# arnauqb/GradABM-JUNE

Hardware: AMD Instinct MI355X
Metric: simulation steps/sec (higher is better)
Workload: dtype f32

## Files before the change

### gradabm-june_amd/csrc/gj_tiled.h

```cpp
#pragma once
#include <hip/hip_runtime.h>
#include <stdint.h>

#include <type_traits>

#include "../../include/gradjune_hip.h"
#include "gj_device.h"

namespace gj {

constexpr int kTileThreads = 1024;
constexpr int kTileWaves = kTileThreads / kWave;
constexpr int kMaxSliceAgents = 19840;
constexpr int kUnroll = 8;
#ifndef GJ_UNROLL_NARROW
#define GJ_UNROLL_NARROW 16
#endif
constexpr int kUnrollNarrow = GJ_UNROLL_NARROW;
#ifndef GJ_VENUE_UNROLL
#define GJ_VENUE_UNROLL 2
#endif
constexpr int kVenueUnroll = GJ_VENUE_UNROLL;
#ifndef GJ_VENUE_UNROLL_C
#define GJ_VENUE_UNROLL_C GJ_VENUE_UNROLL
#endif
constexpr int kVenueUnrollC = GJ_VENUE_UNROLL_C;
#ifndef GJ_CUM_BATCH
#define GJ_CUM_BATCH 8
#endif
constexpr int kCumBatch = GJ_CUM_BATCH;

typedef unsigned long long fx_t;
template <int BITS>
__device__ __forceinline__ constexpr float fx_max() { return (float)(1ull << (50 - BITS)); }
template <int BITS>
__device__ __forceinline__ fx_t to_fx(float x) {
  constexpr double scale = (double)(1ull << BITS);
  constexpr double magic = 6755399441055744.0;
  const double d = __builtin_fma((double)x, scale, magic);
  return (fx_t)(__double_as_longlong(d) - 0x4338000000000000LL);
}
template <int BITS>
__device__ __forceinline__ float from_fx(fx_t v) {
  return (float)((double)(long long)v * (1.0 / (double)(1ull << BITS)));
}
constexpr float kSaturated = 1.0e30f;
__device__ __forceinline__ void fx_flag(uint32_t* flags, int words, int i, float x) {
  const uint32_t bit = 1u << (i & 31);
  if (!(x < 0.0f)) atomicOr(&flags[i >> 5], bit);
  if (!(x > 0.0f)) atomicOr(&flags[words + (i >> 5)], bit);
}
__device__ __forceinline__ float fx_special(uint32_t pos, uint32_t neg, float v) {
  return (pos & neg) ? __builtin_nanf("") : (pos ? kSaturated : (neg ? -kSaturated : v));
}
template <int BITS>
__device__ __forceinline__ float fx_read(const fx_t* sums, const uint32_t* flags, int words, int i) {
  const uint32_t pos = (flags[i >> 5] >> (i & 31)) & 1u, neg = (flags[words + (i >> 5)] >> (i & 31)) & 1u;
  return fx_special(pos, neg, from_fx<BITS>(sums[i]));
}
constexpr int kFxVenue = 36, kFxAgent = 32;
__device__ __forceinline__ uint32_t abs_bits(float x) { return __float_as_uint(x) & 0x7FFFFFFFu; }
template <int N>
__device__ __forceinline__ uint32_t max_abs_bits(const float (&x)[N]) {
  uint32_t m = 0u;
#pragma unroll
  for (int q = 0; q < N; ++q) m = max(m, abs_bits(x[q]));
  return m;
}
template <int BITS>
constexpr uint32_t fx_limit_bits() { return (uint32_t)(127 + 50 - BITS) << 23; }
constexpr uint32_t kAgentLimitBits = fx_limit_bits<kFxAgent>();
static_assert(kAgentLimitBits == 0x48800000u, "the pattern of fx_max<kFxAgent>() = 262144.0f");

template <typename T>
__device__ __forceinline__ T* elem32(T* base, int idx) {
  using Byte = typename std::conditional<std::is_const<T>::value, const char, char>::type;
  return reinterpret_cast<T*>(reinterpret_cast<Byte*>(base) + (uint64_t)((uint32_t)idx * (uint32_t)sizeof(T)));
}
template <typename T>
__device__ __forceinline__ T at32(const T* base, int idx) { return *elem32(base, idx); }
template <typename T>
__device__ __forceinline__ void put32(T* base, int idx, T v) { *elem32(base, idx) = v; }

typedef float gj_v4f __attribute__((ext_vector_type(4)));
typedef unsigned int gj_v4u __attribute__((ext_vector_type(4)));
typedef unsigned int gj_v2u __attribute__((ext_vector_type(2)));
template <typename T>
__device__ __forceinline__ T at32nt(const T* base, int idx) { return __builtin_nontemporal_load(elem32(base, idx)); }
template <typename T>
__device__ __forceinline__ void put32nt(T* base, int idx, T v) { __builtin_nontemporal_store(v, elem32(base, idx)); }
__device__ __forceinline__ uint4 load_nt(const uint4* p) {
  const gj_v4u v = __builtin_nontemporal_load(reinterpret_cast<const gj_v4u*>(p));
  return make_uint4(v.x, v.y, v.z, v.w);
}
__device__ __forceinline__ float4 load_nt(const float4* p) {
  const gj_v4f v = __builtin_nontemporal_load(reinterpret_cast<const gj_v4f*>(p));
  return make_float4(v.x, v.y, v.z, v.w);
}
__device__ __forceinline__ void store_nt(float4* p, float4 x) {
  gj_v4f v = {x.x, x.y, x.z, x.w};
  __builtin_nontemporal_store(v, reinterpret_cast<gj_v4f*>(p));
}
struct TSetA {
  const uint16_t* a_la;
  const int32_t* tile_sptr;
  const int32_t* tile_jpos;
  const int32_t* chunk_ptr;
  const int4* chunk_desc;
  float* val;
  int32_t J;
  int32_t active;
  int32_t raw;
  int32_t wide;
  int32_t direct;
  int32_t presum;
  const int32_t* multi_slots;
};

struct TileAArgs {
  TSetA sets[GJ_MAX_SETS];
  int32_t n_sets;
  int32_t slice_agents;
  int64_t n_agents;
  const float* trans;
// ... 245 lines not shown
    const int i = G.edge_clamped(c0, u, lane);
    la[u] = at32(T.a_la, i);
    sl[u] = at32(slots, i);
  }
}
template <int kU>
__device__ __forceinline__ void scatter_explicit(const TSetA& T, const float* lds_x, int s, int wave, int lane) {
  const Segment G(T, s);
  for (int c0 = wave * kU; c0 < G.n_chunks; c0 += kTileWaves * kU) {
    int la[kU], sl[kU];
    explicit_stage1<kU>(T, G, c0, lane, la, sl);
#pragma unroll
    for (int u = 0; u < kU; ++u)
      if (G.has(c0, u, lane)) put32(T.val, sl[u], lds_x[la[u]]);
  }
}

template <int kU>
__device__ __forceinline__ void gather_explicit(const TSetA& T, fx_t* lds_acc, uint32_t* lds_flags, int flag_words, int s,
                                                int wave, int lane) {
  const Segment G(T, s);
  for (int c0 = wave * kU; c0 < G.n_chunks; c0 += kTileWaves * kU) {
    int la[kU], sl[kU];
    explicit_stage1<kU>(T, G, c0, lane, la, sl);
    float x[kU];
#pragma unroll
    for (int u = 0; u < kU; ++u) x[u] = at32(T.val, sl[u]);
#pragma unroll
    for (int u = 0; u < kU; ++u) x[u] = G.has(c0, u, lane) ? x[u] : 0.0f;
    agent_add_batch<kU>(lds_acc, lds_flags, flag_words, la, x);
  }
}

#ifndef GJ_SCATTER_WAVES_PER_SIMD
#define GJ_SCATTER_WAVES_PER_SIMD 4
#endif
__global__ __launch_bounds__(kTileThreads, GJ_SCATTER_WAVES_PER_SIMD) void k_tile_scatter(const TileAArgs A) {
  extern __shared__ __align__(16) float lds_x[];
  const int tid = threadIdx.x;
  const int wave = __builtin_amdgcn_readfirstlane(tid / kWave), lane = tid % kWave;
  const int s = blockIdx.x;
  const int64_t base = (int64_t)s * A.slice_agents;
  const int n_local = (int)min((int64_t)A.slice_agents, A.n_agents - base);
  const bool two_sources = A.qtrans != A.trans;
  for (int pass = 0; pass < 2; ++pass) {
    if (pass == 1 && !two_sources) break;
    bool any = false;
    for (int t = 0; t < A.n_sets; ++t)
      if (A.sets[t].active && !A.sets[t].presum && (!two_sources || A.sets[t].raw == pass)) any = true;
    if (!any) continue;
    if (pass == 1) __syncthreads();
    load_slice(lds_x, pass == 0 ? A.qtrans : A.trans, base, n_local, tid);
    __syncthreads();
    for (int t = 0; t < A.n_sets; ++t) {
      const TSetA& T = A.sets[t];
      if (!T.active || T.presum || (two_sources && T.raw != pass)) continue;
      if (T.wide == 2) {
        scatter_explicit<kUnroll>(T, lds_x, s, wave, lane);
      } else if (T.wide) {
        scatter_set<true>(T, lds_x, s, wave, lane);
      } else {
        scatter_set<false>(T, lds_x, s, wave, lane);
      }
    }
  }
}

struct TSetB {
  const int32_t* blk_v0;
  const int32_t* blk_e0;
  const uint16_t* e_lv;
  const uint8_t* e_cls;
  float* val;
  const float* v_pc;
  float* cum;
  int32_t stride;
  int32_t nk;
  float beta[GJ_MAX_NETS_PER_SET];
  int32_t table[GJ_MAX_NETS_PER_SET];
  int32_t age75[GJ_MAX_NETS_PER_SET];
  int32_t leisure;
  int32_t direct;
  uint32_t term_limit;
  int32_t _pad_b;
  const uint16_t* pv_blk;
  const int32_t* blk_r0;
  const float* x;
  int64_t n_x;
};

struct TileBArgs {
  TSetB sets[GJ_MAX_SETS];
  const int32_t* work;
  const float* tables;
  int32_t day_type;
  int32_t mode;
  int32_t transpose;
  int32_t _pad;
};

struct ClassWeights {
  float l, lw;
};
__device__ __forceinline__ ClassWeights class_weights(const float* tables, int table, int age75, int day_type, int c) {
  const float l = tables[(int64_t)table * GJ_TABLE_SIZE + day_type * 200 + c];
  return {l, age75 ? l * (((c % 100) > 75) ? 1.0f : 0.0f) : l};
}
template <bool TRANSMITTING, bool RECEIVING, typename TSet>
__device__ __forceinline__ void fill_class_weights(float* transmitting, float* receiving, const TSet& T, const float* tables,
                                                   int day_type, int transpose, int tid) {
  for (int i = tid; i < T.nk * 200; i += kTileThreads) {
    const int k = i / 200, c = i % 200;
    const ClassWeights w = class_weights(tables, T.table[k], T.age75[k], day_type, c);
    if (TRANSMITTING) transmitting[i] = transpose ? w.lw : w.l;
    if (RECEIVING) receiving[i] = transpose ? w.l : w.lw;
  }
}

__device__ __noinline__ void venue_group_slow(fx_t* sums, uint32_t* vflags, int words, uint32_t limit, int base_k, int l0,
                                              int l1, int l2, int l3, int l4, int l5, int l6, int l7, float x0, float x1,
                                              float x2, float x3, float x4, float x5, float x6, float x7) {
  const int lv[8] = {l0, l1, l2, l3, l4, l5, l6, l7};
  const float x[8] = {x0, x1, x2, x3, x4, x5, x6, x7};
#pragma unroll
  for (int q = 0; q < 8; ++q) {
    if (lv[q] == 0xFFFF) continue;
    if (abs_bits(x[q]) <= limit) {
      atomicAdd(&sums[base_k + lv[q]], to_fx<kFxVenue>(x[q]));
    } else {
      fx_flag(vflags, words, base_k + lv[q], x[q]);
    }
  }
}

__device__ __forceinline__ int class_byte(uint32_t four, int j) { return (four >> (8 * j)) & 0xFF; }

struct Group8 {
  uint32_t w[4], c[2];
  float v[8];
  __device__ __forceinline__ Group8(uint4 raw, uint2 craw, float4 xa = make_float4(0.0f, 0.0f, 0.0f, 0.0f),
                                    float4 xb = make_float4(0.0f, 0.0f, 0.0f, 0.0f))
      : w{raw.x, raw.y, raw.z, raw.w}, c{craw.x, craw.y}, v{xa.x, xa.y, xa.z, xa.w, xb.x, xb.y, xb.z, xb.w} {}
  __device__ __forceinline__ int lv(int q) const { return (w[q >> 1] >> ((q & 1) * 16)) & 0xFFFF; }
  __device__ __forceinline__ float x(int q) const { return v[q]; }
  __device__ __forceinline__ int cls(int q) const { return class_byte(c[q >> 2], q & 3); }
  __device__ __forceinline__ void drop(int q) { w[q >> 1] |= 0xFFFFu << ((q & 1) * 16); }
  __device__ __forceinline__ bool one_venue() const {
    return (w[0] == w[1]) && (w[1] == w[2]) && (w[2] == w[3]) && ((w[0] >> 16) == (w[0] & 0xFFFFu)) && (lv(0) != 0xFFFF);
  }
  __device__ __forceinline__ Group8 weighted(const float* tk) const {
    Group8 g = *this;
#pragma unroll
    for (int q = 0; q < 8; ++q) g.v[q] = tk[cls(q)] * v[q];
    return g;
  }
};

#ifdef GJ_DIAG_STAMPS
constexpr int kDiagVenueSlots = 8192;
__device__ unsigned long long gj_diag_venue[3 * kDiagVenueSlots];
struct VenueStamp {
  unsigned long long t0;
  __device__ VenueStamp() : t0(__builtin_amdgcn_s_memrealtime()) {}
  __device__ ~VenueStamp() {
    if (threadIdx.x == 0 && blockIdx.x < kDiagVenueSlots) {
      gj_diag_venue[3 * blockIdx.x] = t0;
      gj_diag_venue[3 * blockIdx.x + 1] = __builtin_amdgcn_s_memrealtime();
      gj_diag_venue[3 * blockIdx.x + 2] = __builtin_amdgcn_s_getreg((31 << 11) | 20) & 0xF;
    }
  }
};
#else
struct VenueStamp {};
#endif

struct VenueItem {
  const TSetB& T;
  int tid, nk;
  int v0, nv;
  int g0, g1;
  fx_t* sums;
  float* cumf;
  float* tabs;
  uint32_t* vflags;
  int vwords;
  int dummy;
  __device__ __forceinline__ VenueItem(const TSetB& T_, int j, float* lds, int tid_)
      : T(T_), tid(tid_), nk(T_.nk), v0(T_.blk_v0[j]), nv(T_.blk_v0[j + 1] - v0), g0(T_.blk_e0[j] >> 3),
        g1(T_.blk_e0[j + 1] >> 3), sums(reinterpret_cast<fx_t*>(lds)), cumf(lds), tabs(lds + 2 * ((size_t)nk * nv + 64)),
        vflags(reinterpret_cast<uint32_t*>(tabs + (T_.leisure ? 2 * nk * 200 : 0))), vwords((nk * nv + 64 + 31) / 32),
        dummy(nk * nv + (tid_ & 63)) {}
  __device__ __forceinline__ const uint4* lv8() const { return reinterpret_cast<const uint4*>(T.e_lv); }
  __device__ __forceinline__ const uint2* cls8() const { return reinterpret_cast<const uint2*>(T.e_cls); }
  __device__ __forceinline__ float4* val4() const { return reinterpret_cast<float4*>(T.val); }
};

__device__ __forceinline__ void run_sums(const VenueItem& W, const Group8& G, int base_k, fx_t* sums, uint32_t* vflags) {
  const uint32_t kLimit = W.T.term_limit;
  static_assert(kFxVenue == 36, "term_limit is derived from 2^(50 - kFxVenue) (fill_set_b)");
  if (__builtin_expect(max_abs_bits(G.v) > kLimit, 0)) {
    venue_group_slow(sums, vflags, W.vwords, kLimit, base_k, G.lv(0), G.lv(1), G.lv(2), G.lv(3), G.lv(4), G.lv(5),
                     G.lv(6), G.lv(7), G.x(0), G.x(1), G.x(2), G.x(3), G.x(4), G.x(5), G.x(6), G.x(7));
    return;
  }
  fx_t s8 = 0;
#pragma unroll
  for (int q = 0; q < 8; ++q) {
    const fx_t f = to_fx<kFxVenue>(G.x(q));
    const bool first = (q == 0) || (G.lv(q) != G.lv(q - (q > 0)));
    s8 = first ? f : s8 + f;
    const bool last = (q == 7) || (G.lv(q + (q < 7)) != G.lv(q));
    const bool take = last && G.lv(q) != 0xFFFF;
    atomicAdd(&sums[take ? base_k + G.lv(q) : W.dummy], s8);
  }
}
__device__ __forceinline__ bool one_venue_sum(const VenueItem& W, const Group8& G, int target, fx_t* sums) {
  if (__builtin_amdgcn_ballot_w64(max_abs_bits(G.v) > W.T.term_limit) != 0ull) return false;
  fx_t s = 0;
#pragma unroll
  for (int q = 0; q < 8; ++q) s += to_fx<kFxVenue>(G.x(q));
  s = wave_sum<fx_t>(s);
  if ((W.tid & (kWave - 1)) == 0) atomicAdd(&sums[target], s);
  return true;
}

__device__ __forceinline__ void venue_zero(const VenueItem& W, fx_t* sums, uint32_t* vflags) {
  for (int i = W.tid; i < W.nk * W.nv + 64; i += kTileThreads) sums[i] = 0;
  for (int i = W.tid; i < 2 * W.vwords; i += kTileThreads) vflags[i] = 0u;
}

__device__ __forceinline__ void venue_sums_tiled(const VenueItem& W, const float* weights, fx_t* sums, uint32_t* vflags) {
  const TSetB& T = W.T;
  auto add_group = [&](const Group8& G) {
    const bool mine = G.one_venue() && (G.lv(0) == __builtin_amdgcn_readfirstlane(G.lv(0)));
    const bool one_venue = __builtin_amdgcn_ballot_w64(mine) == ~0ull;
    if (!T.leisure) {
      if (!(one_venue && one_venue_sum(W, G, G.lv(0), sums))) run_sums(W, G, 0, sums, vflags);
    } else {
      for (int k = 0; k < W.nk; ++k) {
        const Group8 Gk = G.weighted(weights + k * 200);
        if (!(one_venue && one_venue_sum(W, Gk, k * W.nv + G.lv(0), sums))) run_sums(W, Gk, k * W.nv, sums, vflags);
      }
    }
  };
  for (int g = W.g0 + W.tid; g < W.g1; g += kVenueUnroll * kTileThreads) {
    uint4 raw[kVenueUnroll];
    float4 xa[kVenueUnroll], xb[kVenueUnroll];
    uint2 craw[kVenueUnroll];
#pragma unroll
    for (int u = 0; u < kVenueUnroll; ++u) {
      const int gu = min(g + u * kTileThreads, W.g1 - 1);
      raw[u] = W.lv8()[gu];
      xa[u] = load_nt(W.val4() + 2 * gu);
      xb[u] = load_nt(W.val4() + 2 * gu + 1);
      craw[u] = T.leisure ? W.cls8()[gu] : make_uint2(0u, 0u);
    }
#pragma unroll
    for (int u = 0; u < kVenueUnroll; ++u)
      if (g + u * kTileThreads < W.g1) add_group(Group8(raw[u], craw[u], xa[u], xb[u]));
  }
}

__device__ __forceinline__ void venue_sums_runs(const VenueItem& W, int j, fx_t* sums, uint32_t* vflags) {
  const TSetB& T = W.T;
  const int r0 = T.blk_r0[j], r1 = T.blk_r0[j + 1];
  const uint4* pv8 = reinterpret_cast<const uint4*>(T.pv_blk);
  const float4* x4 = reinterpret_cast<const float4*>(T.x);
  const int ga = r0 >> 3, gb = (r1 + 7) >> 3;
  const int g_in = (int)(T.n_x >> 3);
  for (int g = ga + W.tid; g < gb; g += kVenueUnroll * kTileThreads) {
    uint4 raw[kVenueUnroll];
    float4 xa[kVenueUnroll], xb[kVenueUnroll];
#pragma unroll
    for (int u = 0; u < kVenueUnroll; ++u) {
      const int gu = min(g + u * kTileThreads, gb - 1);
      raw[u] = pv8[gu];
      if (gu < g_in) {
        xa[u] = x4[2 * gu];
        xb[u] = x4[2 * gu + 1];
      } else {
        float t[8];
#pragma unroll
        for (int q = 0; q < 8; ++q) t[q] = ((int64_t)gu * 8 + q < T.n_x) ? T.x[(int64_t)gu * 8 + q] : 0.0f;
        xa[u] = make_float4(t[0], t[1], t[2], t[3]);
        xb[u] = make_float4(t[4], t[5], t[6], t[7]);
      }
    }
#pragma unroll
    for (int u = 0; u < kVenueUnroll; ++u) {
      const int gu = g + u * kTileThreads;
      if (gu >= gb) continue;
      Group8 G(raw[u], make_uint2(0u, 0u), xa[u], xb[u]);
#pragma unroll
      for (int q = 0; q < 8; ++q) {
        const int a = gu * 8 + q;
        if (!(a >= r0 && a < r1)) G.drop(q);
      }
      run_sums(W, G, 0, sums, vflags);
    }
  }
}

__device__ __forceinline__ void venue_cum_write(const VenueItem& W, const fx_t* sums, const uint32_t* vflags, float* cumf) {
  const TSetB& T = W.T;
  for (int l0 = W.tid; l0 < W.nv; l0 += kCumBatch * kTileThreads) {
    float pc[kCumBatch];
#pragma unroll
    for (int u = 0; u < kCumBatch; ++u) pc[u] = T.v_pc[W.v0 + min(l0 + u * kTileThreads, W.nv - 1)];
    for (int k = 0; k < W.nk; ++k) {
      const float beta = T.beta[k];
#pragma unroll
      for (int u = 0; u < kCumBatch; ++u) {
        const int lv = l0 + u * kTileThreads;
        if (lv < W.nv) {
          const float c = (beta * pc[u]) * fx_read<kFxVenue>(sums, vflags, W.vwords, k * W.nv + lv);
          T.cum[(int64_t)(W.v0 + lv) * T.stride + k] = c;
          cumf[2 * (k * W.nv + lv)] = c;
        }
      }
    }
  }
}
__device__ __forceinline__ void venue_cum_read(const VenueItem& W, float* cumf) {
  const TSetB& T = W.T;
  for (int k = 0; k < W.nk; ++k) {
    for (int l0 = W.tid; l0 < W.nv; l0 += kCumBatch * kTileThreads) {
      float c[kCumBatch];
#pragma unroll
      for (int u = 0; u < kCumBatch; ++u)
        c[u] = T.cum[(int64_t)(W.v0 + min(l0 + u * kTileThreads, W.nv - 1)) * T.stride + k];
#pragma unroll
      for (int u = 0; u < kCumBatch; ++u) {
        const int lv = l0 + u * kTileThreads;
        if (lv < W.nv) cumf[2 * (k * W.nv + lv)] = c[u];
      }
    }
  }
}

__device__ __forceinline__ void venue_gather(const VenueItem& W, const float* weights, const float* cumf) {
  const TSetB& T = W.T;
  const int nk = W.nk, nv = W.nv;
  for (int g = W.g0 + W.tid; g < W.g1; g += kVenueUnrollC * kTileThreads) {
    uint4 raw[kVenueUnrollC];
    uint2 craw[kVenueUnrollC];
#pragma unroll
    for (int u = 0; u < kVenueUnrollC; ++u) {
      const int gu = min(g + u * kTileThreads, W.g1 - 1);
      raw[u] = W.lv8()[gu];
      craw[u] = T.leisure ? W.cls8()[gu] : make_uint2(0u, 0u);
    }
#pragma unroll
    for (int u = 0; u < kVenueUnrollC; ++u) {
      const int gu = g + u * kTileThreads;
      if (gu >= W.g1) continue;
      const Group8 G(raw[u], craw[u]);
      float r[8];
      if (!T.leisure) {
#pragma unroll
        for (int q = 0; q < 8; ++q) {
          const int lv = G.lv(q);
          const float c = cumf[2 * (lv != 0xFFFF ? lv : 0)];
          r[q] = (lv != 0xFFFF) ? c : 0.0f;
        }
      } else {
#pragma unroll
        for (int q = 0; q < 8; ++q) {
          const int lv = G.lv(q);
          const int c = G.cls(q);
          const int li = lv != 0xFFFF ? lv : 0;
          float a = 0.0f;
          for (int k = 0; k < nk; ++k) a += weights[k * 200 + c] * cumf[2 * (k * nv + li)];
          r[q] = (lv != 0xFFFF) ? a : 0.0f;
        }
      }
      store_nt(W.val4() + 2 * gu, make_float4(r[0], r[1], r[2], r[3]));
      store_nt(W.val4() + 2 * gu + 1, make_float4(r[4], r[5], r[6], r[7]));
    }
  }
}

#ifndef GJ_VENUE_WAVES_PER_SIMD
#define GJ_VENUE_WAVES_PER_SIMD 4
#endif
__global__ __launch_bounds__(kTileThreads, GJ_VENUE_WAVES_PER_SIMD) void k_tile_venues(const TileBArgs B) {
  extern __shared__ __align__(16) float lds_s[];
  [[maybe_unused]] const VenueStamp gj_stamp;
  const int set = B.work[2 * blockIdx.x], j = B.work[2 * blockIdx.x + 1];
  const TSetB& T = B.sets[set];
  if (T.nk == 0) return;
  const VenueItem W(T, j, lds_s, threadIdx.x);
  if (T.leisure) fill_class_weights<true, true>(W.tabs, W.tabs + W.nk * 200, T, B.tables, B.day_type, B.transpose, W.tid);
  if (B.mode != 2) {
    venue_zero(W, W.sums, W.vflags);
    __syncthreads();
    venue_sums_tiled(W, W.tabs, W.sums, W.vflags);
    if (T.pv_blk) venue_sums_runs(W, j, W.sums, W.vflags);
    __syncthreads();
    venue_cum_write(W, W.sums, W.vflags, W.cumf);
    if (B.mode == 1 || T.direct) return;
  } else {
    if (T.direct) return;
    venue_cum_read(W, W.cumf);
  }
  __syncthreads();
  venue_gather(W, W.tabs + W.nk * 200, W.cumf);
}

constexpr int GJ_MAX_PRESUM = 6;
constexpr int64_t kPresumBad = (int64_t)0x8000000000000000ll;
struct TPSet {
  const uint16_t* ell;
  int64_t plane_stride;
  fx_t* partial;
  int32_t planes, V, stride, nk;
  int32_t group_venues;
  int32_t raw, leisure, _pad;
  int32_t table[GJ_MAX_NETS_PER_SET];
  int32_t age75[GJ_MAX_NETS_PER_SET];
};
struct TilePArgs {
  TPSet sets[GJ_MAX_PRESUM];
  int32_t n_sets;
  int32_t agents_per_wg;
  int64_t n_agents;
  const float* trans;
  const float* qtrans;
  const uint8_t* cls;
  const float* tables;
  int32_t day_type, transpose;
};

constexpr int kPresumQuads = 3;
__device__ __forceinline__ void fx_add_or_poison(fx_t* sums, uint32_t* flags, int i, float x) {
  const bool ok = fabsf(x) <= fx_max<kFxVenue>();
  atomicAdd(&sums[i], to_fx<kFxVenue>(ok ? x : 0.0f));
  if (__builtin_expect(!ok, 0)) atomicOr(&flags[i >> 5], 1u << (i & 31));
}

__global__ __launch_bounds__(kTileThreads) void k_tile_presum(const TilePArgs P) {
  extern __shared__ __align__(16) fx_t lds_p[];
  const int tid = threadIdx.x;
  const int64_t a_begin = (int64_t)blockIdx.x * P.agents_per_wg;
  const int64_t a_end = min(P.n_agents, a_begin + P.agents_per_wg);
  const int n_quads = (int)((max(a_end - a_begin, (int64_t)0) + 3) >> 2);
  for (int t = 0; t < P.n_sets; ++t) {
    const TPSet& T = P.sets[t];
    const int nk = T.nk;
    const float* x = T.raw ? P.trans : P.qtrans;
    for (int v0 = 0; v0 < T.V; v0 += T.group_venues) {
      const int nv = min(T.group_venues, T.V - v0);
      const int n_sums = nv * nk;
      const int dummy = n_sums + (tid & 63);
      float* wtab = reinterpret_cast<float*>(lds_p + n_sums + 64);
      uint32_t* flags = reinterpret_cast<uint32_t*>(wtab + (T.leisure ? nk * 200 : 0));
      __syncthreads();
      for (int i = tid; i < n_sums + 64; i += kTileThreads) lds_p[i] = 0;
      for (int i = tid; i < (n_sums + 64 + 31) / 32; i += kTileThreads) flags[i] = 0u;
      if (T.leisure) fill_class_weights<true, false>(wtab, nullptr, T, P.tables, P.day_type, P.transpose, tid);
      __syncthreads();
      for (int plane = 0; plane < T.planes; ++plane) {
        const uint16_t* ell = T.ell + plane * T.plane_stride + a_begin * 2;
        struct Batch {
          uint4 rows[kPresumQuads];
          float4 xs[kPresumQuads];
          uint32_t cl[kPresumQuads];
        };
        auto load = [&](int b0, Batch& B) {
#pragma unroll
          for (int u = 0; u < kPresumQuads; ++u) {
            const int q = min(b0 + tid + u * kTileThreads, n_quads - 1);
            const int64_t a0 = a_begin + 4 * (int64_t)q;
            B.rows[u] = *reinterpret_cast<const uint4*>(ell + 8 * (int64_t)q);
            if (a0 + 4 <= P.n_agents) {
              B.xs[u] = *reinterpret_cast<const float4*>(x + a0);
            } else {
              B.xs[u] = make_float4(a0 < P.n_agents ? x[a0] : 0.0f, a0 + 1 < P.n_agents ? x[a0 + 1] : 0.0f,
                                    a0 + 2 < P.n_agents ? x[a0 + 2] : 0.0f, 0.0f);
            }
            B.cl[u] = T.leisure ? *reinterpret_cast<const uint32_t*>(P.cls + a0) : 0u;
          }
        };
        auto add = [&](int b0, const Batch& B) {
#pragma unroll
          for (int u = 0; u < kPresumQuads; ++u) {
            const int q = b0 + tid + u * kTileThreads;
            if (q >= n_quads) continue;
            const uint32_t w[4] = {B.rows[u].x, B.rows[u].y, B.rows[u].z, B.rows[u].w};
            const float xv[4] = {B.xs[u].x, B.xs[u].y, B.xs[u].z, B.xs[u].w};
// ... 633 lines not shown
```

### gradabm-june_amd/csrc/gradjune_hip.hip

```cpp
#include <hip/hip_runtime.h>
#include <math.h>
#include <stdint.h>
#include <string.h>

#include "../../include/gradjune_hip.h"
#include "gj_device.h"
#include "gj_tiled.h"
#include "gj_agent.h"
#include "gj_location.h"

namespace gj {

struct SetP1 {
  const int32_t* v_rowptr;
  const int32_t* v_agent;
  const float* v_pc;
  float* cum;
  int32_t stride;
  int32_t nk;
  float beta[GJ_MAX_NETS_PER_SET];
  int32_t table[GJ_MAX_NETS_PER_SET];
  int32_t raw;
  int32_t leisure;
};
// ... 822 lines not shown
  }
  if (R.n_sets == 0 || total == 0) return GJ_OK;
  if (total > INT32_MAX) return GJ_E_RANGE;
  R.total = (int32_t)total;
  return launch(k_presum_reduce, grid_for(total, 0, kWave), kThreads, 0, stream, R);
}

static int tiled_scatter(const gj_plan* plan, const gj_agent_state* st, const gj_step_params* p, const Groups& G,
                         hipStream_t stream) {
  const gj_tiled* T = plan->tiled;
  if (plan->n_ext_agents == 0 || G.n == 0) return GJ_OK;
  TileAArgs A;
  fill_set_a(plan, p, G, A.sets);
  A.n_sets = plan->n_sets;
  A.slice_agents = T->slice_agents;
  A.n_agents = plan->n_ext_agents;
  A.trans = st->transmission;
  A.qtrans = p->has_quarantine ? st->q_transmission : st->transmission;
  const size_t lds = slice_lds(T, sizeof(float));
  int rc = allow_lds(k_tile_scatter, lds);
  if (rc) return rc;
  rc = launch(k_tile_scatter, T->n_slices, kTileThreads, lds, stream, A);
  if (rc) return rc;
  return tiled_presum(plan, st, p, G, stream);
}

static uint32_t venue_term_limit(int32_t max_venue_edges) {
  int e = 14;
  int64_t p2 = 4096;
  while (p2 < (int64_t)max_venue_edges && e > -20) {
    p2 <<= 1;
    --e;
  }
  const float lim = ldexpf(1.0f, e);
  uint32_t bits;
  memcpy(&bits, &lim, sizeof(bits));
  return bits;
}

static int tiled_venues(const gj_plan* plan, const gj_agent_state* st, const gj_step_params* p, const Groups& G, int mode,
                        hipStream_t stream) {
  const gj_tiled* T = plan->tiled;
  if (G.n == 0) return GJ_OK;
  if (T->n_work == 0) return mode == 2 ? GJ_OK : tiled_presum_reduce(plan, p, G, stream);
  TileBArgs B;
  for (int s = 0; s < GJ_MAX_SETS; ++s) B.sets[s] = TSetB{};
  size_t lds = 16;
  for (int g = 0; g < G.n; ++g) {
    const int s = G.set[g];
    const gj_tiled_set& S = T->sets[s];
    const gj_edge_set& E = plan->sets[s];
    TSetB& X = B.sets[s];
    X.blk_v0 = S.blk_v0;
    X.blk_e0 = S.blk_e0;
    X.e_lv = S.e_lv;
    X.e_cls = S.e_cls;
    X.val = S.val;
    X.v_pc = E.v_pcontact;
    X.cum = E.cum;
    X.stride = E.cum_stride;
    X.nk = S.n_blocks > 0 ? G.nk[g] : 0;
    if (uses_presum(plan, s)) X.nk = 0;
    X.direct = S.ell_k != 0;
    const NetGroup C = classify_group(p, G, g);
    X.leisure = C.leisure;
    memcpy(X.beta, C.beta, sizeof(X.beta));
    memcpy(X.table, C.table, sizeof(X.table));
    memcpy(X.age75, C.age75, sizeof(X.age75));
    if (C.leisure && !S.e_cls && E.n_edges > 0) return GJ_E_PLAN;
    if (const int rc = check_group(C)) return rc;
    X.pv_blk = nullptr;
    X.blk_r0 = nullptr;
    X.x = nullptr;
    X.n_x = 0;
    if (S.run_pv_blk && mode != 2) {
      if (X.leisure) return GJ_E_PLAN;
      X.x = (p->has_quarantine && !C.raw) ? st->q_transmission : st->transmission;
      if (!X.x) return GJ_E_NULL;
      if (!aligned16(X.x, S.run_pv_blk)) return GJ_E_PLAN;
      X.pv_blk = S.run_pv_blk;
      X.blk_r0 = S.run_blk_r0;
      X.n_x = plan->n_ext_agents;
    }
    const size_t n_sums = (size_t)X.nk * S.max_block_venues + 64;
    const size_t need = n_sums * sizeof(fx_t) + (X.leisure ? 2 * 200 * (size_t)X.nk : 0) * sizeof(float) +
                        2 * ((n_sums + 31) / 32 * 4);
    X.term_limit = venue_term_limit(S.max_venue_edges);
    if (X.nk && need > lds) lds = need;
  }
  B.work = T->work;
  B.tables = plan->tables;
  B.day_type = p->day_type;
  B.mode = mode;
  B.transpose = p->transpose;
  int rc = allow_lds(k_tile_venues, lds);
  if (rc) return rc;
  rc = launch(k_tile_venues, T->n_work, kTileThreads, lds, stream, B);
  if (rc || mode == 2) return rc;
  return tiled_presum_reduce(plan, p, G, stream);
}

static int tiled_agents(const gj_plan* plan, const gj_agent_state* st, const gj_step_params* p, const Groups& G,
                        const gj_step_io* io, int sample, hipStream_t stream) {
  const gj_tiled* T = plan->tiled;
  if (plan->n_agents == 0) return GJ_OK;
  TileDArgs D;
  fill_set_a(plan, p, G, D.sets);
  D.n_sets = plan->n_sets;
  D.slice_agents = T->slice_agents;
  D.n_agents = plan->n_agents;
  D.stage = st->current_stage;
  D.susceptibility = st->susceptibility;
  D.is_infected = st->is_infected;
  D.infection_time = st->infection_time;
  D.not_infected_probs = io ? io->not_infected_probs : nullptr;
  D.new_infected = io ? io->new_infected : nullptr;
  D.trans_susc = io ? io->trans_susc : nullptr;
  D.agent_sums = io ? io->agent_sums : nullptr;
  D.exp_noise = io ? io->exp_noise : nullptr;
  D.now = p->now;
  D.dt = p->delta_time;
  D.q_thr = p->q_threshold;
  D.has_q = p->has_quarantine;
  D.sample = sample;
  D.seed = p->seed;
  D.step = p->step;
  D.agent_offset = p->agent_offset;
  D.clock = p->clock;
  D.acc_scratch = T->agent_scratch;
  size_t lds = agents_lds(T);
  D.n_direct = 0;
  D.day_type = p->day_type;
  D.transpose = p->transpose;
  D.cls = plan->agent_class;
  D.tables = plan->tables;
  const int64_t owned_slices = (plan->n_agents + T->slice_agents - 1) / T->slice_agents;
  for (int g = 0; g < G.n; ++g) {
    const int s = G.set[g];
    const gj_tiled_set& S = T->sets[s];
    const gj_edge_set& E = plan->sets[s];
    const bool run = S.run_pv_win != nullptr;
    if ((!S.ell_k && !run) || S.n_blocks == 0 || E.n_edges == 0) continue;
    if (D.n_direct == GJ_MAX_DIRECT) return GJ_E_PLAN;
    TDirect& X = D.direct[D.n_direct++];
    X.ell = run ? S.run_pv_win : S.ell;
    X.cum = E.cum;
    X.planes = run ? 1 : S.ell_k / 2;
    X.plane_stride = owned_slices * (int64_t)T->slice_agents * 2;
    X.V = run ? S.run_max_window : (int32_t)E.n_venues;
    X.win_lo = run ? S.run_win_lo : nullptr;
    X.win_n = run ? S.run_win_n : nullptr;
    if (run && (uintptr_t)S.run_pv_win % 8 != 0) return GJ_E_PLAN;
    X.stride = E.cum_stride;
    const NetGroup C = classify_group(p, G, g);
    X.nk = C.nk;
    X.raw = C.raw;
    X.leisure = C.leisure;
    memcpy(X.table, C.table, sizeof(X.table));
    memcpy(X.age75, C.age75, sizeof(X.age75));
    if (C.leisure && !classes_by_dword(plan)) return GJ_E_PLAN;
    if (const int rc = check_group(C)) return rc;
  }
  D.table_floats = D.table1_floats = 0;
  D._pad3 = 0;
  if (D.n_direct) {
    const int64_t budget = 160 * 1024 / 4 - 2 * kClassWeightFloats - 2 * kWave;
    int64_t largest = 0;
    for (int t = 0; t < D.n_direct; ++t) {
// ... 735 lines not shown
```

### gradabm-june_amd/grad_june_amd/plan.py

```python
from __future__ import annotations

import os

import ctypes as C
from dataclasses import dataclass, field
from typing import Dict, List, Optional, Sequence

import numpy as np
import torch

from . import _native as N
from . import tiling as TL

LONG_CHUNK = 8192
MAX_ROWS_PER_BLOCK = 2048


@dataclass
class HostEdgeSet:
    name: str
    n_venues: int
    n_edges: int
    v_rowptr: Optional[np.ndarray]
    v_agent: Optional[np.ndarray]
    v_pcontact: np.ndarray
    a_rowptr: Optional[np.ndarray]
    a_venue: Optional[np.ndarray]
    tiled: Optional[TL.TiledEdgeSet] = None
    max_venue_edges: int = 0
    max_agent_edges: int = 0


def p_contact(people) -> np.ndarray:
    people = torch.as_tensor(np.asarray(people)) if not isinstance(people, torch.Tensor) else people.cpu()
    pc = torch.clamp(1.0 / (people - 1), max=1.0)
    pc = torch.clamp(pc, min=0.0)
    return pc.to(torch.float32).numpy()


def _csr(rows: np.ndarray, cols: np.ndarray, n_rows: int):
    order = np.argsort(rows, kind="stable")
    counts = np.bincount(rows, minlength=n_rows)
    rowptr = np.zeros(n_rows + 1, dtype=np.int64)
    np.cumsum(counts, out=rowptr[1:])
    return rowptr.astype(np.int32), cols[order].astype(np.int32)


def compile_edge_set(name: str, agent_index, venue_index, people, n_agents: int,
                     n_ext_agents: Optional[int] = None, csr: bool = True) -> HostEdgeSet:
    agent_index = np.asarray(agent_index).astype(np.int64, copy=False).ravel()
    venue_index = np.asarray(venue_index).astype(np.int64, copy=False).ravel()
    n_ext = n_agents if n_ext_agents is None else n_ext_agents
    n_venues = int(len(people))
    E = int(agent_index.shape[0])
    if E >= 2**31 or n_ext >= 2**31 or n_venues >= 2**31:
        raise ValueError("edge set exceeds int32 indexing")
    if E:
        if agent_index.min() < 0 or agent_index.max() >= n_ext:
            raise ValueError(f"{name}: agent index out of range")
        if venue_index.min() < 0 or venue_index.max() >= n_venues:
            raise ValueError(f"{name}: venue index out of range")
    owned = agent_index < n_agents
    mve = int(np.bincount(venue_index, minlength=1).max()) if E else 0
    mae = int(np.bincount(agent_index[owned], minlength=1).max()) if E and owned.any() else 0
    if not csr:
        return HostEdgeSet(name, n_venues, E, None, None, p_contact(people), None, None, max_venue_edges=mve,
                           max_agent_edges=mae)
    v_rowptr, v_agent = _csr(venue_index, agent_index, n_venues)
    a_rowptr, a_venue = _csr(agent_index[owned], venue_index[owned], n_agents)
    return HostEdgeSet(name, n_venues, E, v_rowptr, v_agent, p_contact(people), a_rowptr, a_venue, max_venue_edges=mve,
                       max_agent_edges=mae)


def _host(a) -> np.ndarray:
    if hasattr(a, "detach"):
        return a.detach().cpu().numpy()
    return np.asarray(a)


def _edge_set_on_device(name: str, es: dict, n_ext: int, n_agents: Optional[int] = None) -> HostEdgeSet:
    people = _host(es["people"])
    n_venues = int(len(people))
    E = int(es["agent"].numel() if hasattr(es["agent"], "numel") else np.asarray(es["agent"]).size)
    if E >= 2**31 or n_ext >= 2**31 or n_venues >= 2**31:
        raise ValueError("edge set exceeds int32 indexing")
    mve = mae = 0
    if E and isinstance(es["venue"], torch.Tensor):
        mve = int(torch.bincount(es["venue"].reshape(-1), minlength=1).max())
        a = es["agent"].reshape(-1)
        if n_agents is not None:
            a = a[a < n_agents]
        mae = int(torch.bincount(a, minlength=1).max()) if a.numel() else 0
    elif E:
        mve = int(np.bincount(np.asarray(es["venue"]).ravel(), minlength=1).max())
        a = np.asarray(es["agent"]).ravel()
        a = a[a < (n_ext if n_agents is None else n_agents)]
        mae = int(np.bincount(a, minlength=1).max()) if len(a) else 0
    return HostEdgeSet(name, n_venues, E, None, None, p_contact(people), None, None, max_venue_edges=mve, max_agent_edges=mae)
# ... 134 lines not shown
                                           pv_blk=a[r + "pv_blk"], pv_win=a[r + "pv_win"], blk_r0=a[r + "blk_r0"],
                                           win_lo=a[r + "win_lo"], win_n=a[r + "win_n"], max_window=int(a[r + "meta"][1]))
        sets.append(hs)
    return HostPlan(int(a["meta/n_agents"]), int(a["meta/n_ext_agents"]), sets, a["agent_class"], a["blocks"],
                    a["long_rows"], int(a["meta/n_partial_slots"]), {s.name: i for i, s in enumerate(sets)},
                    layout=str(a["meta/layout"]), n_slices=int(a["meta/n_slices"]),
                    slice_agents=int(a["meta/slice_agents"]), work=a.get("work"))


def agent_class_of(age, sex) -> np.ndarray:
    age = np.asarray(age).astype(np.int64)
    sex = np.asarray(sex).astype(np.int64)
    if age.size and (age.min() < 0 or age.max() > 99 or sex.min() < 0 or sex.max() > 1):
        raise ValueError("age must be in 0..99 and sex in {0,1} (leisure tables are [2,2,100])")
    return (sex * 100 + age).astype(np.uint8)


def compile_plan(n_agents: int, edge_sets: Dict[str, dict], age=None, sex=None,
                 n_ext_agents: Optional[int] = None, block_order: str = "interleave",
                 layout: str = "csr", leisure_sets: Sequence[str] = ("leisure",),
                 sv_max: int = TL.SV_MAX, eb_target: Optional[int] = None, slices=None, tile_pad: int = 1,
                 nets_per_set: Optional[Dict[str, int]] = None, progress=None,
                 desc_wide: Optional[bool] = None, device=None, direct=None, runs=None, presum=None,
                 desc_explicit: Optional[bool] = None, multi_net_block_div: Optional[int] = None) -> HostPlan:
    if len(edge_sets) > N.GJ_MAX_SETS:
        raise ValueError(f"at most {N.GJ_MAX_SETS} edge sets")
    if layout not in ("csr", "tiled", "both"):
        raise ValueError(layout)
    n_ext = n_agents if n_ext_agents is None else n_ext_agents
    want_csr, want_tiled = layout in ("csr", "both"), layout in ("tiled", "both")
    cls_all = None if age is None else agent_class_of(age, sex)
    S, SA = slices if slices is not None else TL.choose_slices(n_ext)
    if eb_target is None:
        eb_target = TL.choose_block_edges(S)
    if multi_net_block_div is None:
        multi_net_block_div = int(os.environ.get("GJ_MULTI_NET_BLOCK_DIV", "1"))
    if want_tiled and n_ext != n_agents and (-(-n_agents // SA)) * SA > n_ext:
        raise ValueError("halo agents must start on a slice boundary (pad the owned range to a multiple of SA)")
    sets, all_blocks, all_long, work = [], [], [], []
    slot = 0
    n_presum = 0
    for sid, (name, es) in enumerate(edge_sets.items()):
        if device is not None and not want_csr:
            hs = _edge_set_on_device(name, es, n_ext, n_agents)
        else:
            hs = compile_edge_set(name, _host(es["agent"]), _host(es["venue"]), _host(es["people"]), n_agents, n_ext,
                                  csr=want_csr)
        sets.append(hs)
        if want_tiled:
            k = (nets_per_set or {}).get(name, 6 if name in leisure_sets else 1)
            use_cls = cls_all if (name in leisure_sets and cls_all is not None) else None
            forced_run = runs is not None and runs is not False and name in runs
            plan_direct = None
            if not forced_run:
                plan_direct = _direct_plan(name, es, hs.n_venues, n_agents, SA, k, direct, device)
            rf, es_t = None, es
            if runs is not False and (forced_run or (plan_direct is None and runs is None)) and k == 1 \
                    and name not in leisure_sets:
                rf, es_t = _split_runs(name, es, n_agents, hs.n_venues, SA, device, forced_run)
            if device is not None and tile_pad > 1:
                raise NotImplementedError("tile_pad is an experiment of the numpy compile (compile_plan without device=)")
            eb_set = eb_target if k <= 1 else max(8192, eb_target // max(1, multi_net_block_div))
            if device is not None:
                from .tiling_native import build_tiled_native

                hs.tiled = build_tiled_native(name, es_t["agent"], es_t["venue"], hs.n_venues, hs.v_pcontact, S, SA,
                                              agent_class=use_cls, sv_max=max(16, sv_max // max(1, k)),
                                              eb_target=eb_set, wide=desc_wide, device=device, n_ext_agents=n_ext,
                                              explicit=desc_explicit)
            else:
                hs.tiled = TL.build_tiled(name, es_t["agent"], es_t["venue"], hs.n_venues, hs.v_pcontact, S, SA,
                                          agent_class=use_cls, sv_max=max(16, sv_max // max(1, k)),
                                          eb_target=eb_set, wide=desc_wide, explicit=desc_explicit,
                                          tile_pad=tile_pad)
            t = hs.tiled
            if rf is not None:
                t.runs = _finish_runs(rf, t, n_agents, SA, device)
            elif plan_direct is not None:
                t.ell, t.ell_k = plan_direct()
                t.presum = presum is True and plan_direct.all_owned and n_presum < 6
                n_presum += int(t.presum)
            blk_e0, blk_v0 = _host(t.blk_e0).astype(np.int64), _host(t.blk_v0).astype(np.int64)
            prim = np.diff(_host(t.runs.blk_r0).astype(np.int64)) if t.runs is not None else np.zeros(t.n_blocks, np.int64)
            for j in range(t.n_blocks):
                work.append((int(blk_e0[j + 1] - blk_e0[j]) + int(blk_v0[j + 1] - blk_v0[j]) + int(prim[j]), sid, j))
        if progress:
            progress(f"compiled edge set {name}")
        if not want_csr:
            continue
        b, lr, ns = build_schedule(hs.v_rowptr, sid, slot)
        slot += ns
        all_blocks.append(b)
        all_long.append(lr)
    blocks = np.concatenate(all_blocks) if all_blocks else np.zeros((0, 8), np.int32)
    long_rows = np.concatenate(all_long) if all_long else np.zeros((0, 4), np.int32)
    if block_order == "interleave" and len(blocks):
        order = np.argsort(-(blocks[:, 5] - blocks[:, 4]), kind="stable")
        blocks = blocks[order]
    if age is None:
        cls = np.zeros(n_ext, dtype=np.uint8)
    else:
        cls = cls_all
        if len(cls) != n_ext:
            raise ValueError("age/sex must cover owned + halo agents")
    if want_tiled and sum(s.max_agent_edges for s in sets) > TL.MAX_AGENT_EDGES:
        raise ValueError(f"an agent with more than {TL.MAX_AGENT_EDGES} edges: its pass-2 sum (64-bit fixed point, terms "
                         f"up to 262 144) could leave the 64 bits")
    work.sort(key=lambda w: -w[0])
    order = os.environ.get("GJ_WORK_ORDER", "heavy")
    if order == "light":
        work.reverse()
    elif order == "mixed":
        h, l = work[: (len(work) + 1) // 2], work[(len(work) + 1) // 2:][::-1]
        work = [w for pair in zip(h, l + [None] * (len(h) - len(l))) for w in pair if w is not None]
    elif order == "set":
        work.sort(key=lambda w: (w[1], w[2]))
    elif order.startswith("stagger") and len(work) > 512:
        n_light = int(order[7:] or 85)
        light, rest = work[len(work) - n_light:], work[: len(work) - n_light]
        first, later = rest[: 256 - n_light], rest[256 - n_light:]
        mixed, li = [], 0
        step = max(1, len(first) // max(1, n_light))
        for i, w in enumerate(first):
            mixed.append(w)
            if (i + 1) % step == 0 and li < len(light):
                mixed.append(light[li])
                li += 1
        work = mixed + later + light[li:]
    work_arr = np.array([(w[1], w[2]) for w in work], dtype=np.int32).reshape(-1, 2)
    return HostPlan(n_agents, n_ext, sets, cls, np.ascontiguousarray(blocks), long_rows, slot,
                    {s.name: i for i, s in enumerate(sets)}, layout=layout,
                    n_slices=S if want_tiled else 0, slice_agents=SA if want_tiled else 0,
                    work=work_arr if want_tiled else None)


def _direct_plan(name: str, es: dict, n_venues: int, n_agents: int, slice_agents: int, nets: int, direct, device):
    n_edges = int(es["agent"].numel() if hasattr(es["agent"], "numel") else np.asarray(es["agent"]).size)
    if direct is False or n_edges == 0:
        return None
    n_owned_slices = max(1, -(-n_agents // slice_agents))
    builder = None
    if device is not None:
        from .tiling_native import EllBuilder

        builder = EllBuilder(es["agent"], es["venue"], n_venues, n_agents, slice_agents, device)
        e_owned, dmax = builder.degrees()
    else:
        agent = np.asarray(_host(es["agent"]), dtype=np.int64).ravel()
        venue = _host(es["venue"])
        own = agent[agent < n_agents]
        e_owned = int(len(own))
        dmax = int(np.bincount(own, minlength=max(1, n_agents)).max()) if e_owned else 0
    ok = TL.direct_eligible(n_venues, e_owned, n_agents, dmax, nets, slice_agents)
    forced = direct is not None and name in direct
    if forced and not ok:
        raise ValueError(f"edge set {name}: not eligible for the direct form of pass 2")
    if not ok or (direct is not None and not forced):
        return None
    build = (lambda: builder.build(dmax)) if builder is not None else (
        lambda: TL.build_ell(agent, venue, n_agents, n_owned_slices, slice_agents))
    build.all_owned = e_owned == n_edges
    return build


def _split_runs(name: str, es: dict, n_agents: int, n_venues: int, slice_agents: int, device, forced: bool):
    min_share = 0.0 if forced else TL.RUN_MIN_SHARE
    if device is not None:
        from .tiling_native import split_primary_runs_native
# ... 214 lines not shown
```

Before: 2029.

## Fuse multi-network leisure venue sums with class-major padded weight tables

For leisure edge sets with two or more networks, the transmitting class weights are now stored class-major and padded to four or eight floats. This lets each edge group load all network weights for its classes as float4 and accumulate every network in one pass, instead of re-reading the group once per network. Fixed-point conversion constants are pinned in registers, and a per-set maximum weight decides the slow overflow path up front. The host work-cost estimate now weights edges by network count to balance the block schedule. The cost is extra LDS for the padded table and more register pressure in the fused loop.

```diff
diff --git a/gradabm-june_amd/csrc/gj_tiled.h b/gradabm-june_amd/csrc/gj_tiled.h
--- a/gradabm-june_amd/csrc/gj_tiled.h
+++ b/gradabm-june_amd/csrc/gj_tiled.h
@@ -40,6 +40,21 @@
   const double d = __builtin_fma((double)x, scale, magic);
   return (fx_t)(__double_as_longlong(d) - 0x4338000000000000LL);
 }
+template <int BITS>
+struct FxConsts {
+  double scale, magic;
+  static __device__ __forceinline__ FxConsts make() {
+    FxConsts c = {(double)(1ull << BITS), 6755399441055744.0};
+#if defined(__HIP_DEVICE_COMPILE__)
+    asm volatile("" : "+s"(c.scale));
+    asm volatile("" : "+v"(c.magic));
+#endif
+    return c;
+  }
+  __device__ __forceinline__ fx_t to_fx(float x) const {
+    return (fx_t)(__double_as_longlong(__builtin_fma((double)x, scale, magic)) - 0x4338000000000000LL);
+  }
+};
 template <int BITS>
 __device__ __forceinline__ float from_fx(fx_t v) {
   return (float)((double)(long long)v * (1.0 / (double)(1ull << BITS)));
@@ -451,7 +466,7 @@
   int32_t leisure;
   int32_t direct;
   uint32_t term_limit;
-  int32_t _pad_b;
+  int32_t multinet;
   const uint16_t* pv_blk;
   const int32_t* blk_r0;
   const float* x;
@@ -475,14 +490,20 @@
   const float l = tables[(int64_t)table * GJ_TABLE_SIZE + day_type * 200 + c];
   return {l, age75 ? l * (((c % 100) > 75) ? 1.0f : 0.0f) : l};
 }
+__host__ __device__ __forceinline__ constexpr int class_pad(int nk) { return nk <= 4 ? 4 : 8; }
+static_assert(GJ_MAX_NETS_PER_SET <= 8, "class_pad: a class's weights are one or two float4");
 template <bool TRANSMITTING, bool RECEIVING, typename TSet>
 __device__ __forceinline__ void fill_class_weights(float* transmitting, float* receiving, const TSet& T, const float* tables,
-                                                   int day_type, int transpose, int tid) {
+                                                   int day_type, int transpose, int tid, int by_class = 0) {
   for (int i = tid; i < T.nk * 200; i += kTileThreads) {
     const int k = i / 200, c = i % 200;
     const ClassWeights w = class_weights(tables, T.table[k], T.age75[k], day_type, c);
-    if (TRANSMITTING) transmitting[i] = transpose ? w.lw : w.l;
+    if (TRANSMITTING) transmitting[by_class ? c * by_class + k : i] = transpose ? w.lw : w.l;
     if (RECEIVING) receiving[i] = transpose ? w.l : w.lw;
+  }
+  if (TRANSMITTING && by_class > T.nk) {
+    const int n_pad = by_class - T.nk;
+    for (int i = tid; i < n_pad * 200; i += kTileThreads) transmitting[(i / n_pad) * by_class + T.nk + i % n_pad] = 0.0f;
   }
 }
 
@@ -550,14 +571,17 @@
   int g0, g1;
   fx_t* sums;
   float* cumf;
+  int wpad;
   float* tabs;
+  float* tabs2;
   uint32_t* vflags;
   int vwords;
   int dummy;
   __device__ __forceinline__ VenueItem(const TSetB& T_, int j, float* lds, int tid_)
       : T(T_), tid(tid_), nk(T_.nk), v0(T_.blk_v0[j]), nv(T_.blk_v0[j + 1] - v0), g0(T_.blk_e0[j] >> 3),
-        g1(T_.blk_e0[j + 1] >> 3), sums(reinterpret_cast<fx_t*>(lds)), cumf(lds), tabs(lds + 2 * ((size_t)nk * nv + 64)),
-        vflags(reinterpret_cast<uint32_t*>(tabs + (T_.leisure ? 2 * nk * 200 : 0))), vwords((nk * nv + 64 + 31) / 32),
+        g1(T_.blk_e0[j + 1] >> 3), sums(reinterpret_cast<fx_t*>(lds)), cumf(lds), wpad(T_.multinet ? class_pad(nk) : 0),
+        tabs(lds + 2 * (((size_t)nk * nv + 64 + 1) & ~(size_t)1)), tabs2(tabs + (T_.leisure ? (wpad ? wpad : nk) * 200 : 0)),
+        vflags(reinterpret_cast<uint32_t*>(tabs2 + (T_.leisure ? nk * 200 : 0))), vwords((nk * nv + 64 + 31) / 32),
         dummy(nk * nv + (tid_ & 63)) {}
   __device__ __forceinline__ const uint4* lv8() const { return reinterpret_cast<const uint4*>(T.e_lv); }
   __device__ __forceinline__ const uint2* cls8() const { return reinterpret_cast<const uint2*>(T.e_cls); }
@@ -593,6 +617,80 @@
   return true;
 }
 
+__device__ __noinline__ void multi_group_slow(fx_t* sums, uint32_t* vflags, int words, uint32_t limit, int nv, int k0, int k1,
+                                              const float* tabs, int wpad, uint32_t w0, uint32_t w1, uint32_t w2, uint32_t w3,
+                                              uint32_t c0, uint32_t c1, float x0, float x1, float x2, float x3, float x4,
+                                              float x5, float x6, float x7) {
+  const Group8 G(make_uint4(w0, w1, w2, w3), make_uint2(c0, c1), make_float4(x0, x1, x2, x3), make_float4(x4, x5, x6, x7));
+  for (int k = k0; k < k1; ++k) {
+#pragma unroll
+    for (int q = 0; q < 8; ++q) {
+      if (G.lv(q) == 0xFFFF) continue;
+      const float x = tabs[G.cls(q) * wpad + k] * G.x(q);
+      if (abs_bits(x) <= limit) {
+        atomicAdd(&sums[k * nv + G.lv(q)], to_fx<kFxVenue>(x));
+      } else {
+        fx_flag(vflags, words, k * nv + G.lv(q), x);
+      }
+    }
+  }
+}
+__device__ __forceinline__ float max_class_weight(const float* tabs, int n, int tid) {
+  uint32_t m = 0u;
+  for (int i = tid & (kWave - 1); i < n; i += kWave) m = max(m, abs_bits(tabs[i]));
+#pragma unroll
+  for (int off = kWave / 2; off > 0; off >>= 1) m = max(m, (uint32_t)__shfl_xor((int)m, off, kWave));
+  return __uint_as_float(__builtin_amdgcn_readfirstlane(m));
+}
+__device__ __forceinline__ void multi_sums(const VenueItem& W, const Group8& G, bool one_venue, const float* tabs, float wmax,
+                                           const FxConsts<kFxVenue> C, fx_t* sums, uint32_t* vflags) {
+  const uint32_t kLimit = W.T.term_limit;
+  const bool careful = !(abs_bits(__uint_as_float(max_abs_bits(G.v)) * wmax) <= kLimit);
+  const bool wave_run = one_venue && __builtin_amdgcn_ballot_w64(careful) == 0ull;
+  int lv[8];
+  bool first[8], take[8];
+#pragma unroll
+  for (int q = 0; q < 8; ++q) lv[q] = G.lv(q);
+#pragma unroll
+  for (int q = 0; q < 8; ++q) {
+    first[q] = (q == 0) || (lv[q] != lv[q - (q > 0)]);
+    take[q] = ((q == 7) || (lv[q + (q < 7)] != lv[q])) && lv[q] != 0xFFFF;
+  }
+  for (int k0 = 0; k0 < W.nk; k0 += 4) {
+    if (__builtin_expect(careful && !wave_run, 0)) {
+      multi_group_slow(sums, vflags, W.vwords, kLimit, W.nv, k0, min(k0 + 4, W.nk), tabs, W.wpad, G.w[0], G.w[1], G.w[2],
+                       G.w[3], G.c[0], G.c[1], G.x(0), G.x(1), G.x(2), G.x(3), G.x(4), G.x(5), G.x(6), G.x(7));
+      continue;
+    }
+    float4 w4[8];
+#pragma unroll
+    for (int q = 0; q < 8; ++q) w4[q] = *reinterpret_cast<const float4*>(tabs + G.cls(q) * W.wpad + k0);
+#pragma unroll
+    for (int kk = 0; kk < 4; ++kk) {
+      if (k0 + kk >= W.nk) break;
+      const int base_k = __builtin_amdgcn_readfirstlane((k0 + kk) * W.nv);
+      float x[8];
+#pragma unroll
+      for (int q = 0; q < 8; ++q) x[q] = (kk == 0 ? w4[q].x : kk == 1 ? w4[q].y : kk == 2 ? w4[q].z : w4[q].w) * G.x(q);
+      if (wave_run) {
+        fx_t s = 0;
+#pragma unroll
+        for (int q = 0; q < 8; ++q) s += C.to_fx(x[q]);
+        s = wave_sum<fx_t>(s);
+        if ((W.tid & (kWave - 1)) == 0) atomicAdd(&sums[base_k + lv[0]], s);
+      } else {
+        fx_t s8 = 0;
+#pragma unroll
+        for (int q = 0; q < 8; ++q) {
+          const fx_t f = C.to_fx(x[q]);
+          s8 = first[q] ? f : s8 + f;
+          if (take[q]) atomicAdd(&sums[base_k + lv[q]], s8);
+        }
+      }
+    }
+  }
+}
+
 __device__ __forceinline__ void venue_zero(const VenueItem& W, fx_t* sums, uint32_t* vflags) {
   for (int i = W.tid; i < W.nk * W.nv + 64; i += kTileThreads) sums[i] = 0;
   for (int i = W.tid; i < 2 * W.vwords; i += kTileThreads) vflags[i] = 0u;
@@ -600,11 +698,15 @@
 
 __device__ __forceinline__ void venue_sums_tiled(const VenueItem& W, const float* weights, fx_t* sums, uint32_t* vflags) {
   const TSetB& T = W.T;
+  const float wmax = T.multinet ? max_class_weight(weights, 200 * W.wpad, W.tid) : 0.0f;
+  const FxConsts<kFxVenue> fxc = FxConsts<kFxVenue>::make();
   auto add_group = [&](const Group8& G) {
     const bool mine = G.one_venue() && (G.lv(0) == __builtin_amdgcn_readfirstlane(G.lv(0)));
     const bool one_venue = __builtin_amdgcn_ballot_w64(mine) == ~0ull;
     if (!T.leisure) {
       if (!(one_venue && one_venue_sum(W, G, G.lv(0), sums))) run_sums(W, G, 0, sums, vflags);
+    } else if (T.multinet) {
+      multi_sums(W, G, one_venue, weights, wmax, fxc, sums, vflags);
     } else {
       for (int k = 0; k < W.nk; ++k) {
         const Group8 Gk = G.weighted(weights + k * 200);
@@ -759,7 +861,7 @@
   const TSetB& T = B.sets[set];
   if (T.nk == 0) return;
   const VenueItem W(T, j, lds_s, threadIdx.x);
-  if (T.leisure) fill_class_weights<true, true>(W.tabs, W.tabs + W.nk * 200, T, B.tables, B.day_type, B.transpose, W.tid);
+  if (T.leisure) fill_class_weights<true, true>(W.tabs, W.tabs2, T, B.tables, B.day_type, B.transpose, W.tid, W.wpad);
   if (B.mode != 2) {
     venue_zero(W, W.sums, W.vflags);
     __syncthreads();
@@ -773,7 +875,7 @@
     venue_cum_read(W, W.cumf);
   }
   __syncthreads();
-  venue_gather(W, W.tabs + W.nk * 200, W.cumf);
+  venue_gather(W, W.tabs2, W.cumf);
 }
 
 constexpr int GJ_MAX_PRESUM = 6;
diff --git a/gradabm-june_amd/csrc/gradjune_hip.hip b/gradabm-june_amd/csrc/gradjune_hip.hip
--- a/gradabm-june_amd/csrc/gradjune_hip.hip
+++ b/gradabm-june_amd/csrc/gradjune_hip.hip
@@ -928,8 +928,10 @@
       X.blk_r0 = S.run_blk_r0;
       X.n_x = plan->n_ext_agents;
     }
+    X.multinet = X.leisure && X.nk >= 2;
     const size_t n_sums = (size_t)X.nk * S.max_block_venues + 64;
-    const size_t need = n_sums * sizeof(fx_t) + (X.leisure ? 2 * 200 * (size_t)X.nk : 0) * sizeof(float) +
+    const size_t weights = !X.leisure ? 0 : 200 * ((size_t)(X.multinet ? class_pad(X.nk) : X.nk) + (size_t)X.nk);
+    const size_t need = ((n_sums + 1) & ~(size_t)1) * sizeof(fx_t) + weights * sizeof(float) +
                         2 * ((n_sums + 31) / 32 * 4);
     X.term_limit = venue_term_limit(S.max_venue_edges);
     if (X.nk && need > lds) lds = need;
diff --git a/gradabm-june_amd/grad_june_amd/plan.py b/gradabm-june_amd/grad_june_amd/plan.py
--- a/gradabm-june_amd/grad_june_amd/plan.py
+++ b/gradabm-june_amd/grad_june_amd/plan.py
@@ -14,6 +14,7 @@
 
 LONG_CHUNK = 8192
 MAX_ROWS_PER_BLOCK = 2048
+WORK_NET_COST = 0.15
 
 
 @dataclass
@@ -314,8 +315,10 @@
                 n_presum += int(t.presum)
             blk_e0, blk_v0 = _host(t.blk_e0).astype(np.int64), _host(t.blk_v0).astype(np.int64)
             prim = np.diff(_host(t.runs.blk_r0).astype(np.int64)) if t.runs is not None else np.zeros(t.n_blocks, np.int64)
+            net_cost = float(os.environ.get("GJ_WORK_NET_COST", WORK_NET_COST))
             for j in range(t.n_blocks):
-                work.append((int(blk_e0[j + 1] - blk_e0[j]) + int(blk_v0[j + 1] - blk_v0[j]) + int(prim[j]), sid, j))
+                work.append((int((blk_e0[j + 1] - blk_e0[j]) * (1.0 + net_cost * (k - 1))) + int(blk_v0[j + 1] - blk_v0[j])
+                             + int(prim[j]), sid, j))
         if progress:
             progress(f"compiled edge set {name}")
         if not want_csr:
```

New measurement: 2098, median of 6. +3.4%, better.
